# NVlabs/STEP

Hardware: NVIDIA H100
Metric: clips/sec (T=32,224x224) STEP max_iter=3 (higher is better)
Workload: dtype f16

## Files before the change

### include/step_b200.h

```cpp
#ifndef STEP_B200_H_
#define STEP_B200_H_

#include <stddef.h>
#include <stdint.h>

#ifdef __cplusplus
extern "C" {
#endif

typedef struct CUstream_st* step_stream_t;

enum { STEP_F32 = 0, STEP_F16 = 1 };
enum { STEP_OK = 0, STEP_E_ARG = 10001, STEP_E_UNSUPPORTED = 10002, STEP_E_WORKSPACE = 10003,
       STEP_E_DRIVER = 10004 };

int step_version(void);
const char* step_last_error(void);
uint64_t step_launch_count(void);

size_t step_nms_workspace_bytes(int n);
int step_nms_f32(const float* boxes , const float* scores , int n, float thr, int ge,
                 int64_t* keep_out , int* n_keep, void* workspace, size_t ws_bytes,
                 step_stream_t stream);
int step_nms_segmented_f32(const float* boxes, const float* scores, const int* seg_offsets, int n_seg,
// ... 81 lines not shown
  long long noise;
} step_aug_erase;
int step_frames_to_clip_aug_u8(const step_frame_src* table, const step_clip_aug* params, const step_aug_erase* erase,
                               const float* noise, int B, int T, int H, int W, int scale_mode, const float* mean3,
                               const float* std3, float* out, step_stream_t stream);

enum { STEP_A_AUTO = 0, STEP_A_LINEAR = 1, STEP_A_BOX = 2, STEP_A_IM2COL = 3, STEP_A_HALO = 4, STEP_A_BEST = 5,
       STEP_A_SIMT = 9 };
typedef struct {
  int dtype;
  int N, T, H, W;
  int Cin, in_ld;
  int Cout, out_ld, out_coff;
  int KT, KH, KW;
  int ST, SH, SW;
  int PT, PH, PW;
  int OT, OH, OW;
  int relu;
  int w_ld;
  const void* x;
  const void* w;
  const float* scale;
  const float* shift;
  const void* residual;
  int res_ld, res_coff;
  void* y;
  int a_mode;
  int n_splits;
  int split[2];
  void* y_extra[2];
  int ld_extra[2];
  int coff_extra[2];
  int zero_cin_last_kt;
} step_conv_params;
int step_conv3d_fwd(const step_conv_params* p, step_stream_t stream);
int step_debug_tma_tile(const step_conv_params* p, int m_tile, int kt, int kh, int kw, int c0, void* out, int* bk_out,
                        int* box_out, step_stream_t stream);

int step_maxpool3d_fwd(const void* x, int dtype, int N, int T, int H, int W, int C, int in_ld, int KT,
                       int KH, int KW, int ST, int SH, int SW, int PT, int PH, int PW, int pad_hi_t,
                       int pad_hi_h, int pad_hi_w, int OT, int OH, int OW, void* y, int out_ld,
                       step_stream_t stream);
int step_mean_mid(const void* x, int dtype, int A, int B, int P, int C, int ld, void* y, int out_dtype,
                  step_stream_t stream);
int step_mean_mid_strided(const void* x, int dtype, int A, int B, int P, int C, int ld, long long a_stride, void* y,
                          int out_dtype, step_stream_t stream);
size_t step_linear_small_n_workspace_bytes(int M, int K, int N);
int step_linear_small_n(const void* x, int dtype, int M, int K, int x_ld, const void* w, const float* bias,
                        int N, float* y, int y_ld, int act, int accumulate, const int32_t* row_map,
                        void* workspace, size_t ws_bytes, step_stream_t stream);

int step_head_regress(const void* x, int dtype, int R, int T, int K, int x_ld, const void* w12, const float* bias12,
                      int s0, int s1, int e0, int e1, float* local_loc, float* first, float* last, void* workspace,
                      size_t ws_bytes, step_stream_t stream);

int step_bottleneck_exit_f16(const void* h, long long h_ld, const void* w3, const void* x, long long x_ld, const void* w1,
                             const float* shift2, int relu2, void* y, long long y_ld, void* z, long long z_ld, long long M,
                             int planes, int inplanes, int outplanes, step_stream_t stream);

int step_head_losses_f32(const float* logits, const float* local_loc, const float* first_loc, const float* last_loc,
                         const float* tubes, const float* targets, int N, int cls, int T_len, int T, int Tc, float w_loc,
                         float w_nb, float* loss_cls, float* loss_loc, float* loss_nb, int* flags, float* dlogits,
                         float* dloc, float* dfirst, float* dlast, float* scratch, step_stream_t stream);
int step_cls_loss_f32(const float* logits, const float* targets, int N, int cls, float* loss_cls, int* flags, float* dlogits,
                      step_stream_t stream);
int step_roi_align_bwd_nhwc(const void* grad_out, int dtype, int out_ld, const float* rois, int R, float scale, int ph,
// ... 233 lines not shown
```

### step_b200/csrc/conv_umma.cu

```cuda
#include <cuda.h>
#include <stdlib.h>
#include <string.h>

#include "common.cuh"
#include "umma_ptx.cuh"

namespace step {

constexpr int kBM = 128;
constexpr int kMaxBN = 256;
constexpr int kStages = 8;
constexpr int kThreads = 384;
constexpr int kConsumers = 256;
constexpr int kCopyThreads = 96;
constexpr int kPersistMaxKBlocks = 100;
constexpr int kBookBytes = 2 * kStages * 8 + 2 * 8 + 2 * 2 * kMaxBN * 4;
constexpr int kProducerRegs = 40, kConsumerRegs = 232;

#define STEP_CONV_TILES(X)                                                                                         \
  X(64, 32) X(64, 64) X(64, 128) X(64, 144) X(64, 152) X(64, 176) X(64, 192) X(64, 208) X(64, 224) X(64, 256)      \
  X(32, 64) X(32, 128) X(32, 144) X(32, 152) X(32, 160) X(32, 208) X(32, 224)                                      \
  X(16, 64)

__host__ __device__ constexpr int staging_pitch(int BN) { return ((BN / 8 + 1) | 1) * 16; }

struct ConvGeom {
  int mode;
  int taps, KT, KH, KW, PT, PH, PW;
  int kblocks_per_tap;
  int BN, n_tiles;
  int n_stages;
  int n_splits, split[2], ld_extra[2], coff_extra[2];
  __half* y_extra[2];
  int Cout, out_ld, out_coff, res_ld, res_coff, relu;
  int OT, OH, OW, Nimg;
  long long M;
  int tiles;
  int bw, bh, bt, tiles_w, tiles_h, tiles_t;
  int a_bytes;
};

__device__ __forceinline__ long long tile_row_pixel(const ConvGeom& g, int m_tile, int row) {
  if (g.mode == STEP_A_BOX) {
    int r = m_tile;
    const int bw0 = (r % g.tiles_w) * g.bw; r /= g.tiles_w;
    const int bh0 = (r % g.tiles_h) * g.bh; r /= g.tiles_h;
    const int bt0 = (r % g.tiles_t) * g.bt; const int bn = r / g.tiles_t;
    const int dw = row % g.bw, rr = row / g.bw;
    const int dh = rr % g.bh, dt = rr / g.bh;
    const int ow = bw0 + dw, oh = bh0 + dh, ot = bt0 + dt;
    if (dt < g.bt && ow < g.OW && oh < g.OH && ot < g.OT) return (((long long)bn * g.OT + ot) * g.OH + oh) * g.OW + ow;
    return -1;
  }
  const long long m = (long long)m_tile * kBM + row;
  return m < g.M ? m : -1;
}

__device__ __forceinline__ bool mbar_try_wait(uint64_t* bar, uint32_t parity) {
  uint32_t done;
  asm volatile("{\n\t.reg .pred p;\n\tmbarrier.try_wait.parity.shared::cta.b64 p, [%1], %2;\n\tselp.u32 %0, 1, 0, p;\n\t}"
               : "=r"(done) : "r"(smem_u32(bar)), "r"(parity) : "memory");
  return done != 0;
}

template <int BK, int BN>
__global__ void __launch_bounds__(kThreads, 1)
conv_umma_kernel(const __grid_constant__ CUtensorMap map_a, const __grid_constant__ CUtensorMap map_b, ConvGeom g,
                 const float* __restrict__ scale, const float* __restrict__ shift, const __half* __restrict__ residual,
                 __half* __restrict__ y) {
  static_assert(BN % 8 == 0 && BN <= kMaxBN, "wgmma N is a multiple of 8, at most 256");
  constexpr bool kRealloc = BN > 128;
  constexpr bool kBulkOut = BN > 128;
  constexpr int kABytes = kBM * BK * 2;
  constexpr int kBBytes = BN * BK * 2;
  extern __shared__ __align__(1024) uint8_t smem_raw[];
  uint64_t* full_bar = (uint64_t*)smem_raw;
  uint64_t* empty_bar = full_bar + kStages;
  uint64_t* out_full = empty_bar + kStages;
  uint64_t* out_empty = out_full + 1;
  float* s_consts = (float*)(out_empty + 1);
  uint8_t* smem = (uint8_t*)(((uintptr_t)smem_raw + kBookBytes + 1023) & ~(uintptr_t)1023);
  uint8_t* sA = smem;
  uint8_t* sB = smem + g.n_stages * kABytes;
  uint8_t* stg = smem + g.n_stages * (kABytes + kBBytes);
  constexpr int pitch = staging_pitch(BN);

  const int warp = threadIdx.x >> 5, lane = threadIdx.x & 31;
  const int num_kb = g.taps * g.kblocks_per_tap;

  if (threadIdx.x == 0) {
    prefetch_tensormap(&map_a);
    prefetch_tensormap(&map_b);
    for (int s = 0; s < kStages; ++s) { mbar_init(&full_bar[s], 1); mbar_init(&empty_bar[s], 2); }
    mbar_init(out_full, kConsumers / 32);
    mbar_init(out_empty, kCopyThreads / 32);
    fence_barrier_init();
  }
  auto stage_consts = [&](int n_tile, int buf, int t, int nthr) {
    float* s_scale = s_consts + buf * 2 * kMaxBN;
    float* s_shift = s_scale + kMaxBN;
    for (int i = t; i < BN; i += nthr) {
      const int c = n_tile * BN + i;
      s_scale[i] = (scale && c < g.Cout) ? scale[c] : 1.0f;
      s_shift[i] = (shift && c < g.Cout) ? shift[c] : 0.0f;
    }
  };
  if (threadIdx.x < 128) stage_consts(blockIdx.x % g.n_tiles, 0, threadIdx.x, 128);
  __syncthreads();

  if (warp < 4) {
    if constexpr (kRealloc) setmaxnreg_dec<kProducerRegs>();
    if (warp == 0) {
      if (elect_one()) {
        const uint32_t tx_bytes = (uint32_t)(g.a_bytes + kBBytes);
        int stage = 0; uint32_t phase = 0;
        for (int tile = blockIdx.x; tile < g.tiles; tile += gridDim.x) {
          const int m_tile = tile / g.n_tiles, n0 = (tile - m_tile * g.n_tiles) * BN;
          long long m0 = (long long)m_tile * kBM;
          int bn = 0, bt0 = 0, bh0 = 0, bw0 = 0;
          if (g.mode == STEP_A_BOX) {
            int r = m_tile;
            bw0 = (r % g.tiles_w) * g.bw; r /= g.tiles_w;
            bh0 = (r % g.tiles_h) * g.bh; r /= g.tiles_h;
            bt0 = (r % g.tiles_t) * g.bt; bn = r / g.tiles_t;
          }
          int iw = 0, ih = 0, it = 0, in_ = 0;
          if (g.mode == STEP_A_IM2COL) {
            long long r = m0;
            iw = (int)(r % g.OW); r /= g.OW;
            ih = (int)(r % g.OH); r /= g.OH;
            it = (int)(r % g.OT); in_ = (int)(r / g.OT);
            iw -= g.PW; ih -= g.PH; it -= g.PT;
          }
          int kw = 0, kh = 0, kt = 0;
          for (int tap = 0; tap < g.taps; ++tap) {
            for (int kc = 0; kc < g.kblocks_per_tap; ++kc) {
              mbar_wait(&empty_bar[stage], phase ^ 1);
              mbar_expect_tx(&full_bar[stage], tx_bytes);
              const int c0 = kc * BK;
              uint8_t* a_dst = sA + stage * kABytes;
              if (g.mode == STEP_A_LINEAR) {
                tma_load_2d(&map_a, &full_bar[stage], a_dst, c0, (int)m0);
              } else if (g.mode == STEP_A_BOX) {
                tma_load_5d(&map_a, &full_bar[stage], a_dst, c0, bw0 + kw - g.PW, bh0 + kh - g.PH, bt0 + kt - g.PT, bn);
              } else {
                tma_load_im2col_5d(&map_a, &full_bar[stage], a_dst, c0, iw, ih, it, in_, (uint16_t)kw, (uint16_t)kh,
                                   (uint16_t)kt);
              }
              tma_load_3d(&map_b, &full_bar[stage], sB + stage * kBBytes, c0, tap, n0);
              if (++stage == g.n_stages) { stage = 0; phase ^= 1; }
            }
            if (++kw == g.KW) { kw = 0; if (++kh == g.KH) { kh = 0; ++kt; } }
          }
        }
      }
    } else {
      const int ct = threadIdx.x - 32;
      int i_tile = 0;
      for (int tile = blockIdx.x; tile < g.tiles; tile += gridDim.x, ++i_tile) {
        const int m_tile = tile / g.n_tiles, n0 = (tile - m_tile * g.n_tiles) * BN;
        if (tile + (int)gridDim.x < g.tiles) stage_consts((tile + gridDim.x) % g.n_tiles, (i_tile + 1) & 1, ct, kCopyThreads);
        while (!mbar_try_wait(out_full, i_tile & 1)) __nanosleep(128);
        if constexpr (!kBulkOut) {
          constexpr int cpr = BN / 8;
          constexpr int kUnroll = 4;
          for (int i0 = ct; i0 < kBM * cpr; i0 += kUnroll * kCopyThreads) {
            uint4 val[kUnroll];
#pragma unroll
            for (int u = 0; u < kUnroll; ++u) {
              const int i = i0 + u * kCopyThreads, rr = i / cpr, ch = i - rr * cpr;
              if (i < kBM * cpr) val[u] = *reinterpret_cast<const uint4*>(stg + (size_t)rr * pitch + ch * 16);
            }
#pragma unroll
            for (int u = 0; u < kUnroll; ++u) {
              const int i = i0 + u * kCopyThreads, rr = i / cpr, ch = i - rr * cpr;
              const int col = n0 + ch * 8;
              if (i >= kBM * cpr || col >= g.Cout) continue;
              const long long rp = tile_row_pixel(g, m_tile, rr);
              if (rp < 0) continue;
              __half* dst = y + (size_t)rp * g.out_ld + g.out_coff + col;
              if (g.n_splits > 0 && col >= g.split[0]) {
                const int d = (g.n_splits > 1 && col >= g.split[1]) ? 1 : 0;
                dst = g.y_extra[d] + (size_t)rp * g.ld_extra[d] + g.coff_extra[d] + (col - g.split[d]);
              }
              *reinterpret_cast<uint4*>(dst) = val[u];
            }
          }
          __syncwarp();
          if (lane == 0) mbar_arrive(out_empty);
          continue;
        }
        const int end = min(n0 + BN, g.Cout);
        for (int rr = ct; rr < kBM; rr += kCopyThreads) {
          const long long rp = tile_row_pixel(g, m_tile, rr);
          if (rp < 0) continue;
          for (int col = n0; col < end;) {
            __half* dst = y + (size_t)rp * g.out_ld + g.out_coff + col;
            int next = end;
            if (g.n_splits > 0) {
              if (col >= g.split[0]) {
                const int d = (g.n_splits > 1 && col >= g.split[1]) ? 1 : 0;
                dst = g.y_extra[d] + (size_t)rp * g.ld_extra[d] + g.coff_extra[d] + (col - g.split[d]);
                if (d == 0 && g.n_splits > 1) next = min(end, g.split[1]);
              } else {
                next = min(end, g.split[0]);
              }
            }
            bulk_store(dst, stg + (size_t)rr * pitch + (col - n0) * 2, (uint32_t)(next - col) * 2);
            col = next;
          }
        }
        bulk_commit();
        bulk_wait_read<0>();
        __syncwarp();
        if (lane == 0) mbar_arrive(out_empty);
      }
    }
  } else {
    if constexpr (kRealloc) setmaxnreg_inc<kConsumerRegs>();
    const int wg = (warp >> 2) - 1;
    const int ct = threadIdx.x - 128;
    const uint64_t hi = desc_hi_kmajor<BK>();
    const uint64_t a_lo0 = desc_lo(sA + wg * 64 * BK * 2), b_lo0 = desc_lo(sB);
    const int wrow = wg * 64 + (warp & 3) * 16 + (lane >> 2);
    float acc[BN / 2];
    int stage = 0; uint32_t phase = 0;
    int i_tile = 0;
    for (int tile = blockIdx.x; tile < g.tiles; tile += gridDim.x, ++i_tile) {
      const int m_tile = tile / g.n_tiles, n0 = (tile - m_tile * g.n_tiles) * BN;
#pragma unroll
      for (int i = 0; i < BN / 2; ++i) acc[i] = 0.0f;
      int prev = -1;
      for (int kb = 0; kb < num_kb; ++kb) {
        mbar_wait(&full_bar[stage], phase);
        const uint64_t a_lo = a_lo0 + (uint64_t)(stage * (kABytes >> 4)), b_lo = b_lo0 + (uint64_t)(stage * (kBBytes >> 4));
        wg_fence();
#pragma unroll
        for (int k = 0; k < BK / 16; ++k)
          wgmma_f16<BN>(acc, hi | (a_lo + 2 * k), hi | (b_lo + 2 * k), 1u);
        wg_commit();
        wg_wait<1>();
        if (prev >= 0 && ct % 128 == 0) mbar_arrive(&empty_bar[prev]);
        prev = stage;
        if (++stage == g.n_stages) { stage = 0; phase ^= 1; }
      }
      wg_wait<0>();
      if (ct % 128 == 0) mbar_arrive(&empty_bar[prev]);
      mbar_wait(out_empty, (i_tile & 1) ^ 1);
      const float* s_scale = s_consts + (i_tile & 1) * 2 * kMaxBN;
      const float* s_shift = s_scale + kMaxBN;
#pragma unroll
      for (int i = 0; i < 2; ++i) {
        const int row = wrow + 8 * i;
        const long long pix = residual ? tile_row_pixel(g, m_tile, row) : -1;
        const __half* rrow = pix >= 0 ? residual + (size_t)pix * g.res_ld + g.res_coff + n0 : nullptr;
        uint8_t* srow = stg + (size_t)row * pitch;
#pragma unroll
        for (int j = 0; j < BN / 8; ++j) {
          const int col = 8 * j + 2 * (lane & 3);
          float f0 = fmaf(acc[4 * j + 2 * i], s_scale[col], s_shift[col]);
          float f1 = fmaf(acc[4 * j + 2 * i + 1], s_scale[col + 1], s_shift[col + 1]);
// ... 25 lines not shown
  __syncwarp();
  if (threadIdx.x == 0) {
    long long m0 = (long long)m_tile * kBM;
    mbar_expect_tx(&bar, (uint32_t)g.a_bytes);
    if (g.mode == STEP_A_LINEAR) {
      tma_load_2d(&map_a, &bar, smem, c0, (int)m0);
    } else if (g.mode == STEP_A_BOX) {
      int r = m_tile;
      int bw0 = (r % g.tiles_w) * g.bw; r /= g.tiles_w;
      int bh0 = (r % g.tiles_h) * g.bh; r /= g.tiles_h;
      int bt0 = (r % g.tiles_t) * g.bt; int bn = r / g.tiles_t;
      tma_load_5d(&map_a, &bar, smem, c0, bw0 + kw - g.PW, bh0 + kh - g.PH, bt0 + kt - g.PT, bn);
    } else {
      long long r = m0;
      int iw = (int)(r % g.OW); r /= g.OW;
      int ih = (int)(r % g.OH); r /= g.OH;
      int it = (int)(r % g.OT); int in_ = (int)(r / g.OT);
      tma_load_im2col_5d(&map_a, &bar, smem, c0, iw - g.PW, ih - g.PH, it - g.PT, in_, (uint16_t)kw, (uint16_t)kh, (uint16_t)kt);
    }
  }
  mbar_wait(&bar, 0);
  __syncwarp();
  for (int i = threadIdx.x; i < kABytes / 4; i += 32) ((uint32_t*)out)[i] = ((uint32_t*)smem)[i];
}

static int pick_bk(int Cin) {
  if (Cin <= 16) return 16;
  const int k64 = (Cin + 63) / 64 * 64, k32 = (Cin + 31) / 32 * 32;
  return k32 < k64 ? 32 : 64;
}

struct ConvTile {
  int BK, BN;
  void (*kernel)(CUtensorMap, CUtensorMap, ConvGeom, const float*, const float*, const __half*, __half*);
};
static const ConvTile kTiles[] = {
#define STEP_TILE_ENTRY(bk, bn) {bk, bn, conv_umma_kernel<bk, bn>},
    STEP_CONV_TILES(STEP_TILE_ENTRY)
#undef STEP_TILE_ENTRY
};
constexpr int kNumTiles = (int)(sizeof(kTiles) / sizeof(kTiles[0]));

static int pick_tile(int BK, int Cout) {
  int best = -1; long best_pad = 0, best_n = 0;
  for (int i = 0; i < kNumTiles; ++i) {
    if (kTiles[i].BK != BK) continue;
    const long n = (Cout + kTiles[i].BN - 1) / kTiles[i].BN, pad = n * kTiles[i].BN - Cout;
    if (best < 0 || pad < best_pad || (pad == best_pad && n < best_n)) { best = i; best_pad = pad; best_n = n; }
  }
  return best;
}

static void pick_box(int OW, int OH, int OT, int* bw, int* bh, int* bt) {
  double best = -1;
  for (int w = 1; w <= OW && w <= kBM; ++w)
    for (int h = 1; h <= OH && w * h <= kBM; ++h) {
      int t = kBM / (w * h);
      if (t > OT) t = OT;
      if (t < 1) continue;
      double eff = ((double)OW / (((OW + w - 1) / w) * w)) * ((double)OH / (((OH + h - 1) / h) * h)) *
                   ((double)OT / (((OT + t - 1) / t) * t)) * ((double)(w * h * t) / kBM);
      if (eff > best + 1e-9) { best = eff; *bw = w; *bh = h; *bt = t; }
    }
}

static std::atomic<int> g_two_ctas[kNumTiles];
static std::atomic<unsigned long long> g_attr_seen[kNumTiles];
// ... 115 lines not shown
  }
  if (rc) return rc;
  if ((rc = encode_weights3d(&pl->map_b, p->w, p->Cout, taps, p->Cin, p->w_ld, BK, g.BN, swizzle_for(BK),
                             CU_TENSOR_MAP_L2_PROMOTION_L2_256B, "conv3d(f16): B")))
    return rc;
  STEP_CHECK_ARG(m_tiles * g.n_tiles < (1LL << 31), "conv3d(f16): grid too large");
  g.tiles = (int)(m_tiles * g.n_tiles);
  const long per_stage = (long)kBM * BK * 2 + (long)g.BN * BK * 2;
  const long fixed = kBookBytes + 1024 + (long)kBM * staging_pitch(g.BN);
  int st = (int)((113L * 1024 - fixed) / per_stage);
  if (st > kStages) st = kStages;
  bool two = false;
  if (st >= 3) {
    if (int rc = two_ctas_fit(pl->tile, (size_t)(fixed + st * per_stage), &two)) return rc;
  }
  if (!two) st = (int)((227L * 1024 - fixed) / per_stage);
  g.n_stages = st > kStages ? kStages : st;
  STEP_CHECK_ARG(g.n_stages >= 2, "conv3d(f16): tile does not fit shared memory");
  pl->smem_bytes = (size_t)(fixed + g.n_stages * per_stage);
  int sms = 0;
  if (int rc = sm_count(&sms)) return rc;
  const long resident = (long)sms * (two ? 2 : 1);
  const bool persist = g.taps * g.kblocks_per_tap <= kPersistMaxKBlocks && g.tiles > resident;
  pl->grid = dim3((unsigned)(persist ? resident : g.tiles));
  return 0;
}

int conv3d_umma_launch(const step_conv_params* p, step_stream_t stream) {
  ConvPlan pl;
  if (int rc = build_plan(p, &pl)) return rc;
  const ConvTile& t = kTiles[pl.tile];
  if (int rc = allow_dynamic_smem(t.kernel, g_attr_seen[pl.tile], 227 * 1024, "conv_umma_kernel")) return rc;
  return launch_tc("conv_umma_kernel", t.kernel, pl.grid, kThreads, pl.smem_bytes, cu(stream), pl.map_a, pl.map_b, pl.g,
                   p->scale, p->shift, (const __half*)p->residual, (__half*)p->y);
}

}

using namespace step;

extern "C" int step_debug_tma_tile(const step_conv_params* p, int m_tile, int kt, int kh, int kw, int c0, void* out,
                                   int* bk_out, int* box_out , step_stream_t stream) {
  ConvPlan pl;
  if (int rc = build_plan(p, &pl)) return rc;
  if (bk_out) *bk_out = pl.BK;
  if (box_out) { box_out[0] = pl.g.bw; box_out[1] = pl.g.bh; box_out[2] = pl.g.bt; }
  size_t smem = 1024 + (size_t)kBM * pl.BK * 2;
  if (pl.BK == 64) tma_dump_kernel<64><<<1, 32, smem, cu(stream)>>>(pl.map_a, pl.g, m_tile, kt, kh, kw, c0, (uint8_t*)out);
  else if (pl.BK == 32) tma_dump_kernel<32><<<1, 32, smem, cu(stream)>>>(pl.map_a, pl.g, m_tile, kt, kh, kw, c0, (uint8_t*)out);
  else tma_dump_kernel<16><<<1, 32, smem, cu(stream)>>>(pl.map_a, pl.g, m_tile, kt, kh, kw, c0, (uint8_t*)out);
  STEP_LAUNCH_CHECK("tma_dump_kernel");
  return 0;
}
```

### step_b200/engine.py

```python
import contextlib
import math
import os

import torch

from . import _lib as L

A_MODE = {"box": L.A_BOX, "im2col": L.A_IM2COL, "auto": L.A_AUTO, "simt": L.A_SIMT, "best": L.A_BEST}[
    os.environ.get("STEP_B200_AMODE", "best")]


RECORDER = None
TAPE = None
DEBUG_SYNC = os.environ.get("STEP_B200_DEBUG_SYNC", "0") == "1"
STEM_HALO = os.environ.get("STEP_B200_STEM_HALO", "1") != "0"


BRANCH_STREAMS = os.environ.get("STEP_B200_BRANCH_STREAMS", "1") != "0"
FUSE_1X1 = os.environ.get("STEP_B200_FUSE_1X1", "1") != "0"
_side_streams = {}


@contextlib.contextmanager
def recording(tape):
    global TAPE, BRANCH_STREAMS
    saved = TAPE, BRANCH_STREAMS
    TAPE = tape
    if tape is not None:
        BRANCH_STREAMS = False
    try:
        yield tape
    finally:
        TAPE, BRANCH_STREAMS = saved


def side_streams(device, n=3):
    key = (device.type, device.index, torch.cuda.current_stream(device).cuda_stream)
    st = _side_streams.get(key)
    if st is None or len(st) < n:
        st = [torch.cuda.Stream(device=device) for _ in range(n)]
        _side_streams[key] = st
    return st[:n]


def run_parallel(device, main_fn, side_fns, first_side=0):
    if not BRANCH_STREAMS or not side_fns:
        main_fn()
        for f in side_fns:
            f()
        return
    cur = torch.cuda.current_stream(device)
    fork = cur.record_event()
    streams = side_streams(device, first_side + len(side_fns))[first_side:]
    joins = []
    for st, f in zip(streams, side_fns):
        st.wait_event(fork)
        with torch.cuda.stream(st):
            f()
            joins.append(st.record_event())
    main_fn()
    for ev in joins:
        cur.wait_event(ev)


def torch_dtype(code):
    return torch.float16 if code == L.F16 else torch.float32


def dtype_code(fp16):
    env = os.environ.get("STEP_B200_PRECISION")
    if env:
        return {"fp16": L.F16, "fp32": L.F32}[env]
    return L.F16 if fp16 else L.F32


class Act:
    __slots__ = ("buf", "C", "coff")

    def __init__(self, buf, C=None, coff=0):
        assert buf.dim() == 5 and buf.is_contiguous()
        self.buf = buf
        self.C = buf.shape[4] - coff if C is None else C
        self.coff = coff

    @staticmethod
    def empty(N, T, H, W, C, code, device, ld=None):
        return Act(torch.empty((N, T, H, W, ld or C), dtype=torch_dtype(code), device=device), C, 0)

    N = property(lambda s: s.buf.shape[0])
    T = property(lambda s: s.buf.shape[1])
    H = property(lambda s: s.buf.shape[2])
    W = property(lambda s: s.buf.shape[3])
    ld = property(lambda s: s.buf.shape[4])
    code = property(lambda s: L.dt(s.buf))
    device = property(lambda s: s.buf.device)
# ... 197 lines not shown
        out_dims = same_out_dims((x.T, x.H, x.W), k, stride)
    p = L.step_conv_params()
    p.dtype = code
    p.N, p.T, p.H, p.W = x.N, x.T, x.H, x.W
    p.Cin, p.in_ld = x.C, x.ld
    p.Cout, p.out_ld, p.out_coff = out.C + sum(e.C for e in (extra_outs or [])), out.ld, out.coff
    if extra_outs:
        p.n_splits = len(extra_outs)
        edge = out.C
        for i, e in enumerate(extra_outs):
            p.split[i] = edge
            p.y_extra[i] = e.buf.data_ptr()
            p.ld_extra[i], p.coff_extra[i] = e.ld, e.coff
            edge += e.C
    p.KT, p.KH, p.KW = k
    p.ST, p.SH, p.SW = stride
    p.PT, p.PH, p.PW = pad_lo
    p.OT, p.OH, p.OW = out_dims
    p.relu = 1 if relu else 0
    p.w_ld = w_packed.shape[2]
    p.x = x.data_ptr()
    p.w = w_packed.data_ptr()
    p.scale = scale.data_ptr() if scale is not None else None
    p.shift = shift.data_ptr() if shift is not None else None
    if residual is not None:
        p.residual = residual.buf.data_ptr()
        p.res_ld, p.res_coff = residual.ld, residual.coff
    p.y = out.buf.data_ptr()
    p.zero_cin_last_kt = int(zero_cin_last_kt)
    p.a_mode = A_MODE if a_mode is None else a_mode
    if p.a_mode in (L.A_BOX, L.A_IM2COL, L.A_BEST) and k == (1, 1, 1):
        p.a_mode = L.A_AUTO
    assert (out.N, out.T, out.H, out.W) == (x.N,) + tuple(out_dims), "conv: output buffer shape mismatch"
    L.check(L.lib().step_conv3d_fwd(p, L.stream()))
    if DEBUG_SYNC:
        try:
            torch.cuda.synchronize()
        except Exception:
            print("conv fault:", {f: getattr(p, f) for f, _ in p._fields_ if isinstance(getattr(p, f), int)}, flush=True)
            raise
    if TAPE is not None:
        TAPE.append(dict(kind="conv", x=x, w=w_packed, scale=scale, out=out, extra_outs=list(extra_outs or []), k=tuple(k),
                         stride=tuple(stride), pad_lo=tuple(pad_lo), relu=bool(relu), residual=residual, tag=tag))
    if RECORDER is not None:
        RECORDER.append((p, (x.buf, w_packed, scale, shift, out.buf, residual.buf if residual is not None else None,
                             [e.buf for e in (extra_outs or [])])))
    return out


def pool_out(size, k, s):
    lo, hi = same_pad(k, s)
    P = size + lo + hi
    o = -(-(P - k) // s) + 1
    if (o - 1) * s >= P:
        o -= 1
    return o, lo, hi


def maxpool(x, k, s, out=None):
    (ot, pt, ht), (oh, ph, hh), (ow, pw, hw) = (pool_out(d, kk, ss) for d, kk, ss in zip((x.T, x.H, x.W), k, s))
    if out is None:
        out = Act.empty(x.N, ot, oh, ow, x.C, x.code, x.device)
    L.check(L.lib().step_maxpool3d_fwd(L.c_void_p(x.data_ptr()), x.code, x.N, x.T, x.H, x.W, x.C, x.ld, k[0], k[1],
                                       k[2], s[0], s[1], s[2], pt, ph, pw, ht, hh, hw, ot, oh, ow,
                                       L.c_void_p(out.data_ptr()), out.ld, L.stream()))
    if TAPE is not None:
        TAPE.append(dict(kind="pool", x=x, out=out, k=tuple(k), stride=tuple(s), pad_lo=(pt, ph, pw), pad_hi=(ht, hh, hw)))
    return out


def mean_mid(x_ptr, code, A, B, P, C, ld, device, out_code=L.F32):
    y = torch.empty((A, P * C), dtype=torch_dtype(out_code), device=device)
    L.check(L.lib().step_mean_mid(L.c_void_p(x_ptr), code, A, B, P, C, ld, L.ptr(y), out_code, L.stream()))
    return y


def linear_small_n(x, M, K, x_ld, w, bias, N, y=None, act=0, accumulate=False, row_map=None):
    if y is None:
        y = torch.empty((M, N), dtype=torch.float32, device=x.device)
# ... 7 lines not shown
```

### step_b200/inference.py

```python
import numpy as np
import torch

from . import _lib as L
from . import engine as E
from .engine import Act
from .networks import act_of, to_act
from .tube_utils import flatten_tubes, tube_update


def _ext_mode(args, i):
    if i < args.max_iter and args.NUM_CHUNKS[i + 1] == args.NUM_CHUNKS[i] + 2:
        return {"predict": L.EXT_PREDICT, "extrapolate": L.EXT_EXTRAPOLATE}.get(args.temporal_mode, L.EXT_MEAN)
    return L.EXT_NONE


def stage_tubes(tubes, device):
    flat_np, tubes_nums = flatten_tubes(tubes, batch_idx=True)
    flat = torch.from_numpy(np.ascontiguousarray(flat_np, dtype=np.float32)).to(device)
    clip_of_tube = torch.from_numpy(np.repeat(np.arange(len(tubes_nums)), tubes_nums).astype(np.int32)).to(device)
    return flat, clip_of_tube, tubes_nums


def inference_device(args, feat, ctx_all, nets, exec_iter, flat, clip_of_tube, tubes_nums):
    dev = feat.device
    code = feat.code
    B, T_total = feat.N, feat.T
    R = flat.shape[0]
    roi_net = nets['roi_net']
    history, steps = [], []
    width, height = float(args.image_size[0]), float(args.image_size[1])
    decode_nb = args.temporal_mode == "predict"
    with torch.cuda.device(dev):
        for i in range(1, exec_iter + 1):
            chunks = args.NUM_CHUNKS[i]
            T_start = int((args.NUM_CHUNKS[args.max_iter] - chunks) / 2) * args.T
            T_len = chunks * args.T
            if flat.shape[1] != T_len:
                raise RuntimeError("inference: tubes have %d frames but step %d pools %d" % (flat.shape[1], i, T_len))
            head = nets['det_net%d' % (i - 1)]
            ps = head.pool_size
            cat = Act.empty(R, T_len, ps, ps, 832 + head.fc_dim, code, dev)
            roi_net.pool_into(feat, flat, cat.frames().slice(0, 832), T_len, T_total, T_start)
            ctx_mean = None
            if ctx_all is not None:
                sl = ctx_all[:, T_start:T_start + T_len].contiguous()
                ctx_mean = E.mean_mid(sl.data_ptr(), L.F32, B, T_len, 1, sl.shape[2], sl.shape[2], dev)
            hdev = torch.device(head.device) if getattr(head, "device", None) not in (None, "cpu") else dev
            if hdev.type == "cuda" and hdev.index is None:
                hdev = torch.device("cuda", torch.cuda.current_device())
            if hdev != dev:
                cat_h = Act(cat.buf.to(hdev))
                cm = ctx_mean.to(hdev) if ctx_mean is not None else None
                with torch.cuda.device(hdev):
                    outs = head.forward_act(cat_h, cm, clip_of_tube.to(hdev))
                prob, loc, first, last = (o.to(dev) for o in outs)
            else:
                prob, loc, first, last = head.forward_act(cat, ctx_mean, clip_of_tube)
            ext = _ext_mode(args, i)
            pred_loc, pf, pl, flat_next = tube_update(flat, loc, first if decode_nb else None,
                                                      last if decode_nb else None, clip_of_tube, args.T, decode_nb,
                                                      ext, width, height)
            pred_prob = prob.view(-1, 1, args.num_classes).expand(-1, T_len, -1)
            history.append({'pred_prob': pred_prob, 'pred_loc': pred_loc, 'pred_first_loc': pf, 'pred_last_loc': pl,
                            'tubes_nums': tubes_nums})
            steps.append((flat_next, prob))
            flat = flat_next
    return history, steps


def inference(args, conv_feat, context_feat, nets, exec_iter, tubes, want_trajectory=True):
    L.need_cuda(conv_feat)
    dev = conv_feat.device
    code = E.dtype_code(nets['det_net0'].fp16)
    feat = act_of(conv_feat)
    if feat is None or feat.code != code:
        feat = to_act(conv_feat, code)
    flat, clip_of_tube, tubes_nums = stage_tubes(tubes, dev)
    ctx_all = None
    if not args.no_context:
        L.need_cuda(context_feat)
        ctx_all = context_feat.detach().float().reshape(feat.N, context_feat.shape[1], feat.T).permute(0, 2, 1).contiguous()
    history, steps = inference_device(args, feat, ctx_all, nets, exec_iter, flat, clip_of_tube, tubes_nums)

    trajectory = []
    if want_trajectory:
        for (flat_next, prob), h in zip(steps, history):
            props = flat_next[:, :, 1:].cpu().numpy()
            cls = torch.argmax(prob, dim=-1).cpu()
            T_len = h['pred_loc'].shape[1]
            cur, s = [], 0
            for n in tubes_nums:
                cur.append((props[s:s + n], cls[s:s + n].view(-1, 1).expand(-1, T_len)))
                s += n
            trajectory.append(cur)
    return history, trajectory
```

### step_b200/networks.py

```python
import os

import torch
import torch.nn as nn
import torch.nn.init as init

from . import _lib as L
from . import engine as E
from .engine import Act
from .i3d import build_trunk_stages, set_bn_eval, set_freeze_stats
from .roi_layers import ROIAlign, ROIPool


def weights_init(m):
    if isinstance(m, (nn.Conv2d, nn.Linear, nn.Conv3d)):
        init.xavier_normal_(m.weight.data)
        if m.bias is not None:
            init.constant_(m.bias.data, 0.0)


def act_of(t):
    if t.dim() != 5:
        return None
    phys = t.permute(0, 1, 3, 4, 2)
    if phys.is_contiguous():
# ... 61 lines not shown
                L.ptr(flat_tubes), R, 1.0 / 16.0, ps, ps]
        if self.pool_mode == 'align':
            args.append(0)
        args += [L.c_void_p(out.data_ptr()), out.ld, roi_T, feat_T, t_start]
        if self.pool_mode == 'align':
            args.append(0 if feat.code == L.F16 else 1)
        if argmax is not None:
            args.append(L.ptr(argmax))
        args.append(L.stream())
        L.check(fn(*args))
        return out


class BaseNet(nn.Module):

    def __init__(self, cfg):
        super(BaseNet, self).__init__()
        self.base_name = cfg.base_net
        self.kinetics_pretrain = cfg.kinetics_pretrain
        self.freeze_stats = cfg.freeze_stats
        self.freeze_affine = cfg.freeze_affine
        self.fp16 = cfg.fp16
        if self.base_name == "i3d":
            self.base_model = build_base_i3d(self.kinetics_pretrain, self.freeze_affine)
        else:
            raise NotImplementedError
        set_freeze_stats(self.base_model, self.freeze_stats)

    def forward(self, x):
        L.need_cuda(x)
        with torch.cuda.device(x.device):
            return self.forward_act(x).logical()

    def forward_act(self, x):
        L.need_cuda(x)
        if x.dim() != 5:
            raise RuntimeError("BaseNet: expected [N,T,C,H,W]")
        code = E.dtype_code(self.fp16)
        N, T, C, H, W = x.shape
        src = x.detach().to(torch.float32).contiguous()
        m = self.base_model
        if code == L.F16 and T % 2 == 0 and H % 2 == 0 and W % 2 == 0 and C == 3:
            s2d = Act.empty(N, T // 2, H // 2, W // 2, 32, L.F16, x.device)
            L.check(L.lib().step_clip_to_s2d_f16(L.ptr(src), N, T, C, H, W, L.ptr(s2d.buf), 32, L.stream()))
            a = m[0].forward_s2d(s2d)
        else:
            if code == L.F16:
                raise RuntimeError("BaseNet(fp16): T, H, W must be even and C == 3")
            cp = (C + 3) // 4 * 4
            a = Act.empty(N, T, H, W, cp, code, x.device)
            L.check(L.lib().step_clip_to_ndhwc(L.ptr(src), N, T, C, H, W, L.ptr(a.buf), code, cp, L.stream()))
            a = m[0](a)
        for i in range(1, len(m)):
            a = m[i](a)
        return a

    def train(self, mode=True):
        nn.Module.train(self, mode)
        if mode and self.freeze_stats:
            set_bn_eval(self.base_model)
        return self


def build_base_i3d(kinetics_pretrain=None, freeze_affine=True):
    stages = build_trunk_stages()
    base_model = nn.Sequential(*stages)
# ... 22 lines not shown
```

### step_b200/runner.py

```python
import torch

from . import _lib as L
from . import engine as E
from .inference import inference_device, stage_tubes
from .postprocess import Detector
from .transforms import frame_entry, frame_table


class StepRunner:
    def __init__(self, cfg, nets, B, T_in, H, W, tubes, device=None, context=False, use_graph=True, warmup=2,
                 detect=None, transform=None, source_hw=None):
        self.cfg, self.nets = cfg, nets
        self.device = device or torch.device("cuda", torch.cuda.current_device())
        self.context = context and not cfg.no_context
        self.x = torch.zeros((B, T_in, 3, H, W), dtype=torch.float32, device=self.device)
        self.transform = transform
        if transform is not None:
            if source_hw is None:
                raise ValueError("StepRunner: a transform needs source_hw = (H0, W0)")
            if tuple(transform.size) != (W, H):
                raise ValueError("StepRunner: transform size %s is not the clip's (W, H) = %s" % (transform.size, (W, H)))
            self.src = torch.zeros((B, T_in, 3) + tuple(source_hw), dtype=torch.uint8, device=self.device)
            self.table = frame_table([frame_entry(self.src[b], W) for b in range(B)], self.device)
        self.flat, self.clip_of_tube, self.tubes_nums = stage_tubes(tubes, self.device)
        self.graph = None
        self.history = None
        self.detections = None
        self.detectors = {}
        if detect is not None:
            for i in detect.get("steps", [cfg.max_iter - 1]):
                self.detectors[i] = Detector(self.tubes_nums, cfg.num_classes, self.device, detect["conf_thresh"],
                                             detect["nms_thresh"], W, H, topk=detect.get("topk", 0))
        if not use_graph:
            return
        side = torch.cuda.Stream(device=self.device)
        side.wait_stream(torch.cuda.current_stream(self.device))
        with torch.cuda.stream(side):
            for _ in range(warmup):
                self._body()
        torch.cuda.current_stream(self.device).wait_stream(side)
        torch.cuda.synchronize(self.device)
        g = torch.cuda.CUDAGraph()
        with torch.cuda.graph(g):
            self.history = self._body()
        self.graph = g

    def _body(self):
        with torch.no_grad():
            if self.transform is not None:
                self.transform.launch(self.table, self.x.shape[0], self.x.shape[1], self.x)
            feat = self.nets["base_net"].forward_act(self.x)
            ctx_all = self.nets["context_net"].forward_act(feat) if self.context else None
            hist, _ = inference_device(self.cfg, feat, ctx_all, self.nets, self.cfg.max_iter, self.flat,
                                       self.clip_of_tube, self.tubes_nums)
            if self.detectors:
                self.detections = {i: d.run(hist[i]["pred_prob"], hist[i]["pred_loc"]) for i, d in self.detectors.items()}
        return hist

    def __call__(self, clips=None):
        if self.transform is not None:
            if clips is not None:
                self._stage_frames(clips)
        elif clips is not None and clips.data_ptr() != self.x.data_ptr():
            self.x.copy_(clips, non_blocking=True)
        if self.graph is None:
            return self._body()
        self.graph.replay()
        return self.history

    def _stage_frames(self, frames):
        clips = list(frames) if isinstance(frames, (list, tuple)) else [frames[b] for b in range(frames.shape[0])]
        want = tuple(self.src.shape[1:])
        if len(clips) != self.src.shape[0] or any(tuple(c.shape) != want or c.dtype != torch.uint8 for c in clips):
            raise ValueError("StepRunner: expected %d uint8 clips %s (the captured source size), got %s" % (
                self.src.shape[0], want, [(c.dtype, tuple(c.shape)) for c in clips]))
        if isinstance(frames, torch.Tensor):
            self.src.copy_(frames, non_blocking=True)
        else:
            for dst, c in zip(self.src, clips):
# ... 2 lines not shown
```

### step_b200/training.py

```python
import contextlib
import ctypes

import torch

from . import _lib as L


def head_losses(logits, local_loc, first_loc, last_loc, tubes, targets, T, lambda_reg=5.0, lambda_neighbor=1.0,
                want_grads=False):
    dev = L.same_device(logits, local_loc, first_loc, last_loc, tubes, targets)
    f32 = lambda t: t.detach().to(torch.float32).contiguous()
    logits, local_loc, first_loc, last_loc, tubes, targets = map(f32, (logits, local_loc, first_loc, last_loc, tubes, targets))
    N, cls = logits.shape
    T_len, Tc = local_loc.shape[1], first_loc.shape[1]
    if targets.shape != (N, 3, 6 + cls) or tubes.shape != (N, T_len, 5):
        raise RuntimeError("head_losses: targets %s / tubes %s do not match N=%d, T'=%d, classes=%d"
                           % (tuple(targets.shape), tuple(tubes.shape), N, T_len, cls))
    with torch.cuda.device(dev):
        loss_cls = torch.empty((N * cls,), dtype=torch.float32, device=dev)
        loss_loc = torch.empty((1,), dtype=torch.float32, device=dev)
        loss_nb = torch.empty((1,), dtype=torch.float32, device=dev)
        flags = torch.empty((3,), dtype=torch.int32, device=dev)
        scratch = torch.empty((N * 12,), dtype=torch.float32, device=dev)
        g = None
        if want_grads:
            g = {"logits": torch.empty_like(logits), "local_loc": torch.empty_like(local_loc),
                 "first_loc": torch.empty_like(first_loc), "last_loc": torch.empty_like(last_loc)}
        L.check(L.lib().step_head_losses_f32(L.ptr(logits), L.ptr(local_loc), L.ptr(first_loc), L.ptr(last_loc), L.ptr(tubes),
                                             L.ptr(targets), N, cls, T_len, int(T), Tc, float(lambda_reg), float(lambda_neighbor),
                                             L.ptr(loss_cls), L.ptr(loss_loc), L.ptr(loss_nb), L.ptr(flags),
                                             L.ptr(g["logits"]) if g else None, L.ptr(g["local_loc"]) if g else None,
                                             L.ptr(g["first_loc"]) if g else None, L.ptr(g["last_loc"]) if g else None,
                                             L.ptr(scratch), L.stream()))
        if int(flags[0].item()) == 0:
            loss_cls = torch.zeros((1,), dtype=torch.float32, device=dev)
    return (loss_cls, loss_loc, loss_nb) if not want_grads else (loss_cls, loss_loc, loss_nb, g)


# ... 162 lines not shown
    try:
        yield
    finally:
        e1.record()
        TIMING.setdefault(name, []).append((e0, e1))


def timing_summary():
    torch.cuda.synchronize()
    return {k: round(sum(a.elapsed_time(b) for a, b in v), 2) for k, v in (TIMING or {}).items()}


def trainable_bn(tag):
    bn = getattr(tag, "batch3d", None) if getattr(tag, "use_bn", False) else None
    if bn is None or not (bn.weight.requires_grad or bn.bias.requires_grad):
        return None
    return bn


def check_bn_affine(nets):
    bns = [("%s.%s" % (key, name), m) for key, mod in nets.items() if mod is not None for name, m in mod.named_modules()
           if isinstance(m, torch.nn.BatchNorm3d) and (m.weight.requires_grad or m.bias.requires_grad)]
    if not bns:
        return
    with torch.no_grad():
        bad = torch.stack([((m.weight == 0) & (m.bias > 0)).any() for _, m in bns]).cpu()
    if bool(bad.any()):
        name = bns[int(bad.nonzero()[0, 0])][0]
        raise ValueError("BatchNorm %s has a channel with gamma == 0 and beta > 0: its output is constant and gamma's gradient "
                         "cannot be recovered from it; freeze that layer's affine parameters or give gamma a non-zero value"
                         % name)


def tape_backward(tape, grads, loss_scale=1.0, need_input_grad=None):
    from . import engine as E
    from .engine import Act
    out = {}
    lib = L.lib()
    inv = 1.0 / float(loss_scale)

    def add(param, g):
        out[param] = out[param] + g if param in out else g

    for e in reversed(tape):
        f16 = e["x"].code == L.F16
        if e["kind"] == "pool":
            x, y = e["x"], e["out"]
            gy, gx = grads.of(y), grads.of(x)
            k, s, pl, ph = e["k"], e["stride"], e["pad_lo"], e["pad_hi"]
            ws = torch.empty((y.N * y.T * y.H * y.W * y.C,), dtype=torch.uint8, device=x.device)
            pool_bwd = lib.step_maxpool3d_bwd_f16 if f16 else lib.step_maxpool3d_bwd_f32
            with _phase("pool_bwd"):
                L.check(pool_bwd(L.c_void_p(x.data_ptr()), x.ld, L.c_void_p(gy.data_ptr()), gy.ld, x.N, x.T, x.H,
                                                   x.W, x.C, k[0], k[1], k[2], s[0], s[1], s[2], pl[0], pl[1], pl[2], ph[0], ph[1],
                                                   ph[2], y.T, y.H, y.W, L.c_void_p(gx.data_ptr()), gx.ld, L.ptr(ws), L.stream()))
            continue
        x, w, k = e["x"], e["w"], e["k"]
        strided = e["stride"] != (1, 1, 1)
        if strided and (f16 or need_input_grad is None or need_input_grad(e)):
            raise NotImplementedError("tape_backward: a strided convolution has a weight gradient on the fp32 path only, and no "
                                      "input gradient (the trunk's stem needs none)")
        outs = [e["out"]] + e["extra_outs"]
        y0 = e["out"]
        M = y0.N * y0.T * y0.H * y0.W
        n_total = sum(o.C for o in outs)
        dz = torch.empty((y0.N, y0.T, y0.H, y0.W, n_total), dtype=x.buf.dtype, device=x.device)
# ... 550 lines not shown
```

### step_b200/two_branch.py

```python
import torch
import torch.nn as nn

from . import _lib as L
from . import engine as E
from .engine import Act
from .i3d import I3D_head, set_bn_eval, set_freeze_stats
from .networks import to_act, weights_init

__all__ = ['ContextNet', 'TwoBranchNet']


def build_conv(base_name='i3d', kinetics_pretrain=None, mode='global', freeze_affine=True):
    if base_name != "i3d":
        raise NotImplementedError
    i3d = I3D_head()
    if kinetics_pretrain is not None:
        import os
        if not os.path.isfile(kinetics_pretrain):
            raise ValueError("Kinetics_pretrain doesn't exist: {}".format(kinetics_pretrain))
        model_dict = i3d.state_dict()
        pre = torch.load(kinetics_pretrain, map_location="cpu")
        model_dict.update({k: v for k, v in pre.items() if k in model_dict})
        i3d.load_state_dict(model_dict)
    if mode == 'context':
# ... 60 lines not shown
        self.conv2 = nn.Conv2d(inplanes, planes, kernel_size=1, bias=False)
        self.conv3 = nn.Conv2d(planes, planes, kernel_size=3, stride=stride, padding=1, bias=False)
        self.conv4 = nn.Conv2d(planes, outplanes, kernel_size=1, bias=False)
        self.relu = nn.ReLU(inplace=True)
        self.stride = stride

    def forward(self, x):
        box = {}
        E.run_parallel(x.device,
                       lambda: box.__setitem__("o", conv2d(self.conv3, conv2d(self.conv2, x, True), True)),
                       [lambda: box.__setitem__("res", conv2d(self.conv1, x, False))])
        return conv2d(self.conv4, box["o"], True, residual=box["res"])


class ContextNet(nn.Module):

    def __init__(self, cfg):
        super(ContextNet, self).__init__()
        self.T = cfg.T
        self.freeze_stats = cfg.freeze_stats
        self.freeze_affine = cfg.freeze_affine
        self.fp16 = cfg.fp16
        self.i3d_conv_context = build_conv(cfg.base_net, cfg.kinetics_pretrain, 'context', self.freeze_affine)
        set_freeze_stats(self.i3d_conv_context, self.freeze_stats)
        self.avg_pool = nn.AvgPool3d((1, 13, 13), (1, 1, 1))
        self._init_net()

    def forward(self, conv_feat):
        L.need_cuda(conv_feat)
        with torch.cuda.device(conv_feat.device):
            ctx = self.forward_act(to_act(conv_feat, E.dtype_code(self.fp16)))
        return ctx.permute(0, 2, 1).unsqueeze(-1).unsqueeze(-1)

    def forward_act(self, a, keep=None):
        x = self.i3d_conv_context[0](a)
        x = self.i3d_conv_context[1](x)
        x = self.i3d_conv_context[2](x)
        if keep is not None:
            keep["mixed_5c"] = x
        y = E.mean_mid(x.data_ptr(), x.code, x.N * x.T, x.H * x.W, 1, x.C, x.ld, x.device)
        return y.view(x.N, x.T, x.C)

    def _init_net(self):
        pass

    def set_device(self, device):
        self.device = device

    def train(self, mode=True):
        nn.Module.train(self, mode)
        if mode and self.freeze_stats:
            set_bn_eval(self.i3d_conv_context)
        return self


class TwoBranchNet(nn.Module):

    def __init__(self, cfg, cls_only=False):
        super(TwoBranchNet, self).__init__()
        self.num_classes = cfg.num_classes
        self.T = cfg.T
        self.base_net = cfg.base_net
        self.freeze_stats = cfg.freeze_stats
        self.freeze_affine = cfg.freeze_affine
        self.fc_dim = cfg.fc_dim
        self.dropout_prob = cfg.dropout
# ... 47 lines not shown
    def forward(self, global_feat, context_feat=None, tubes=None, targets=None):
        dev = self.device
        if dev is not None and str(dev) != "cpu":
            global_feat = global_feat.to(dev)
            if context_feat is not None:
                context_feat = context_feat.to(dev)
        L.same_device(global_feat, context_feat)
        code = E.dtype_code(self.fp16)
        N, T, C, W, H = global_feat.shape
        with torch.cuda.device(global_feat.device):
            cat = Act.empty(N, T, W, H, C + self.fc_dim, code, global_feat.device)
            src = to_act(global_feat, code)
            cat.buf[..., :C].copy_(src.buf[..., src.coff:src.coff + C])
            ctx_mean = None
            if context_feat is not None:
                cf = context_feat.detach().float().contiguous().view(N * context_feat.shape[1], T)
                ctx_mean = E.mean_mid(cf.data_ptr(), L.F32, N * context_feat.shape[1], T, 1, 1, 1, cf.device).view(N, -1)
            if targets is None:
                prob, loc, first, last = self.forward_act(cat, ctx_mean, None)
            else:
                prob, loc, first, last, logits = self.forward_act(cat, ctx_mean, None, want_logits=True)
        z = torch.tensor(0., device=prob.device)
        if targets is None:
            return prob, loc, first, last, z.view(-1), z.view(-1), z.view(-1)
        from . import training
        if tubes is None:
            raise RuntimeError("TwoBranchNet.forward: targets need tubes")
        tb, tg = tubes.to(prob.device), targets.to(prob.device)
        if self.cls_only:
            return prob, loc, first, last, training.cls_loss(logits, tg), z.view(-1), z.view(-1)
        lc, ll, ln = training.head_losses(logits, loc, first, last, tb, tg, self.T)
        return prob, loc, first, last, lc, ll, ln

    def forward_act(self, cat, ctx_mean=None, ctx_row_map=None, want_logits=False, keep=None, dropout=None):
        R, T, ps = cat.N, cat.T, self.pool_size
        code = cat.code
        roi = cat.slice(0, 832)
        g = self.i3d_conv[0](roi)
        g = self.i3d_conv[1](g)
        w, bias = _packed(self.downsample, code)
        gconv = cat.slice(832, self.fc_dim)
        E.conv(g, w, None, bias, gconv, (1, 1, 1), relu=False, tag=self.downsample)
        hw = self._head_weights()
        D = self.fc_dim * ps * ps
        gsrc = gconv
        if dropout is not None:
            gsrc = Act.empty(R, T, ps, ps, self.fc_dim, code, cat.device)
            ctx_cols = 0 if hw["ctx_w"] is None else hw["ctx_w"].shape[1]
            L.check(L.lib().step_dropout_global_fwd(dropout[0], L.c_void_p(gconv.data_ptr()), code, cat.ld, R, T, ps * ps, self.fc_dim,
                                                    ctx_cols, L.c_void_p(gsrc.data_ptr()), gsrc.ld, L.stream()))
        xbar = E.mean_mid(gsrc.data_ptr(), code, R, T, ps * ps, self.fc_dim, gsrc.ld, cat.device)
        has_ctx = ctx_mean is not None and hw["ctx_w"] is not None
        logits = E.linear_small_n(xbar, R, D, D, hw["cls_w"], hw["cls_b"], self.num_classes,
                                  act=0 if has_ctx else 1)
        if has_ctx:
            E.linear_small_n(ctx_mean, R, 1024, 1024, hw["ctx_w"], None, self.num_classes, y=logits, act=1,
                             accumulate=True, row_map=ctx_row_map)
        prob = logits
        raw = None
        if want_logits:
            raw = E.linear_small_n(xbar, R, D, D, hw["cls_w"], hw["cls_b"], self.num_classes, act=0)
            if has_ctx:
                E.linear_small_n(ctx_mean, R, 1024, 1024, hw["ctx_w"], None, self.num_classes, y=raw, act=0,
                                 accumulate=True, row_map=ctx_row_map)
        if self.cls_only:
            if keep is not None:
# ... 87 lines not shown
```

Measured before the change: 1162.

## Schedule persistent conv tiles dynamically with a global atomic tile counter

Result: no change. 1169, median of 6 (+0.7%).

```diff
diff --git a/include/step_b200.h b/include/step_b200.h
--- a/include/step_b200.h
+++ b/include/step_b200.h
@@ -137,6 +137,7 @@
   int ld_extra[2];
   int coff_extra[2];
   int zero_cin_last_kt;
+  unsigned int* tile_counter;
 } step_conv_params;
 int step_conv3d_fwd(const step_conv_params* p, step_stream_t stream);
 int step_debug_tma_tile(const step_conv_params* p, int m_tile, int kt, int kh, int kw, int c0, void* out, int* bk_out,
diff --git a/step_b200/csrc/conv_umma.cu b/step_b200/csrc/conv_umma.cu
--- a/step_b200/csrc/conv_umma.cu
+++ b/step_b200/csrc/conv_umma.cu
@@ -14,7 +14,9 @@
 constexpr int kConsumers = 256;
 constexpr int kCopyThreads = 96;
 constexpr int kPersistMaxKBlocks = 100;
-constexpr int kBookBytes = 2 * kStages * 8 + 2 * 8 + 2 * 2 * kMaxBN * 4;
+constexpr int kTileRing = kStages;
+constexpr int kTileReaders = kConsumers / 32 + kCopyThreads / 32;
+constexpr int kBookBytes = 2 * kStages * 8 + 2 * 8 + 2 * 2 * kMaxBN * 4 + 2 * kTileRing * 8 + kTileRing * 4;
 constexpr int kProducerRegs = 40, kConsumerRegs = 232;
 
 #define STEP_CONV_TILES(X)                                                                                         \
@@ -63,11 +65,25 @@
   return done != 0;
 }
 
+__device__ __forceinline__ int next_tile(unsigned int* counter, int tile, int tiles) {
+  if (!counter) return tile + (int)gridDim.x;
+  const int t = (int)gridDim.x + (int)atomicAdd(counter, 1u);
+  if (t >= tiles) {
+    __threadfence();
+    if (atomicAdd(counter + 1, 1u) == gridDim.x - 1) {
+      __threadfence();
+      counter[0] = 0u;
+      counter[1] = 0u;
+    }
+  }
+  return t;
+}
+
 template <int BK, int BN>
 __global__ void __launch_bounds__(kThreads, 1)
 conv_umma_kernel(const __grid_constant__ CUtensorMap map_a, const __grid_constant__ CUtensorMap map_b, ConvGeom g,
                  const float* __restrict__ scale, const float* __restrict__ shift, const __half* __restrict__ residual,
-                 __half* __restrict__ y) {
+                 __half* __restrict__ y, unsigned int* __restrict__ tile_counter) {
   static_assert(BN % 8 == 0 && BN <= kMaxBN, "wgmma N is a multiple of 8, at most 256");
   constexpr bool kRealloc = BN > 128;
   constexpr bool kBulkOut = BN > 128;
@@ -79,6 +95,9 @@
   uint64_t* out_full = empty_bar + kStages;
   uint64_t* out_empty = out_full + 1;
   float* s_consts = (float*)(out_empty + 1);
+  uint64_t* tid_full = (uint64_t*)(s_consts + 2 * 2 * kMaxBN);
+  uint64_t* tid_empty = tid_full + kTileRing;
+  int* tile_ids = (int*)(tid_empty + kTileRing);
   uint8_t* smem = (uint8_t*)(((uintptr_t)smem_raw + kBookBytes + 1023) & ~(uintptr_t)1023);
   uint8_t* sA = smem;
   uint8_t* sB = smem + g.n_stages * kABytes;
@@ -94,8 +113,18 @@
     for (int s = 0; s < kStages; ++s) { mbar_init(&full_bar[s], 1); mbar_init(&empty_bar[s], 2); }
     mbar_init(out_full, kConsumers / 32);
     mbar_init(out_empty, kCopyThreads / 32);
+    for (int s = 0; s < kTileRing; ++s) { mbar_init(&tid_full[s], 1); mbar_init(&tid_empty[s], kTileReaders); }
     fence_barrier_init();
-  }
+    tile_ids[0] = blockIdx.x;
+    mbar_arrive(&tid_full[0]);
+  }
+  auto take_tile = [&](int i) {
+    mbar_wait(&tid_full[i % kTileRing], (uint32_t)(i / kTileRing) & 1);
+    const int t = tile_ids[i % kTileRing];
+    __syncwarp();
+    if (lane == 0) mbar_arrive(&tid_empty[i % kTileRing]);
+    return t;
+  };
   auto stage_consts = [&](int n_tile, int buf, int t, int nthr) {
     float* s_scale = s_consts + buf * 2 * kMaxBN;
     float* s_shift = s_scale + kMaxBN;
@@ -114,7 +143,7 @@
       if (elect_one()) {
         const uint32_t tx_bytes = (uint32_t)(g.a_bytes + kBBytes);
         int stage = 0; uint32_t phase = 0;
-        for (int tile = blockIdx.x; tile < g.tiles; tile += gridDim.x) {
+        for (int i = 0, tile = blockIdx.x, next; tile < g.tiles; ++i, tile = next) {
           const int m_tile = tile / g.n_tiles, n0 = (tile - m_tile * g.n_tiles) * BN;
           long long m0 = (long long)m_tile * kBM;
           int bn = 0, bt0 = 0, bh0 = 0, bw0 = 0;
@@ -152,14 +181,19 @@
             }
             if (++kw == g.KW) { kw = 0; if (++kh == g.KH) { kh = 0; ++kt; } }
           }
+          const int slot = (i + 1) % kTileRing;
+          mbar_wait(&tid_empty[slot], ((uint32_t)((i + 1) / kTileRing) & 1) ^ 1);
+          next = next_tile(tile_counter, tile, g.tiles);
+          tile_ids[slot] = next;
+          mbar_arrive(&tid_full[slot]);
         }
       }
     } else {
       const int ct = threadIdx.x - 32;
-      int i_tile = 0;
-      for (int tile = blockIdx.x; tile < g.tiles; tile += gridDim.x, ++i_tile) {
+      for (int i_tile = 0, tile = take_tile(0), next; tile < g.tiles; ++i_tile, tile = next) {
         const int m_tile = tile / g.n_tiles, n0 = (tile - m_tile * g.n_tiles) * BN;
-        if (tile + (int)gridDim.x < g.tiles) stage_consts((tile + gridDim.x) % g.n_tiles, (i_tile + 1) & 1, ct, kCopyThreads);
+        next = take_tile(i_tile + 1);
+        if (next < g.tiles) stage_consts(next % g.n_tiles, (i_tile + 1) & 1, ct, kCopyThreads);
         while (!mbar_try_wait(out_full, i_tile & 1)) __nanosleep(128);
         if constexpr (!kBulkOut) {
           constexpr int cpr = BN / 8;
@@ -225,8 +259,9 @@
     const int wrow = wg * 64 + (warp & 3) * 16 + (lane >> 2);
     float acc[BN / 2];
     int stage = 0; uint32_t phase = 0;
-    int i_tile = 0;
-    for (int tile = blockIdx.x; tile < g.tiles; tile += gridDim.x, ++i_tile) {
+    for (int i_tile = 0;; ++i_tile) {
+      const int tile = take_tile(i_tile);
+      if (tile >= g.tiles) break;
       const int m_tile = tile / g.n_tiles, n0 = (tile - m_tile * g.n_tiles) * BN;
 #pragma unroll
       for (int i = 0; i < BN / 2; ++i) acc[i] = 0.0f;
@@ -318,7 +353,7 @@
 
 struct ConvTile {
   int BK, BN;
-  void (*kernel)(CUtensorMap, CUtensorMap, ConvGeom, const float*, const float*, const __half*, __half*);
+  void (*kernel)(CUtensorMap, CUtensorMap, ConvGeom, const float*, const float*, const __half*, __half*, unsigned int*);
 };
 static const ConvTile kTiles[] = {
 #define STEP_TILE_ENTRY(bk, bn) {bk, bn, conv_umma_kernel<bk, bn>},
@@ -500,7 +535,7 @@
   const ConvTile& t = kTiles[pl.tile];
   if (int rc = allow_dynamic_smem(t.kernel, g_attr_seen[pl.tile], 227 * 1024, "conv_umma_kernel")) return rc;
   return launch_tc("conv_umma_kernel", t.kernel, pl.grid, kThreads, pl.smem_bytes, cu(stream), pl.map_a, pl.map_b, pl.g,
-                   p->scale, p->shift, (const __half*)p->residual, (__half*)p->y);
+                   p->scale, p->shift, (const __half*)p->residual, (__half*)p->y, p->tile_counter);
 }
 
 }
diff --git a/step_b200/engine.py b/step_b200/engine.py
--- a/step_b200/engine.py
+++ b/step_b200/engine.py
@@ -1,4 +1,5 @@
 import contextlib
+import functools
 import math
 import os
 
@@ -61,6 +62,42 @@
     main_fn()
     for ev in joins:
         cur.wait_event(ev)
+
+
+COUNTER_SLOTS = 512
+_counters = None
+
+
+@contextlib.contextmanager
+def tile_counters():
+    global _counters
+    if _counters is not None:
+        yield
+        return
+    _counters = {}
+    try:
+        yield
+    finally:
+        _counters = None
+
+
+def counted(fn):
+    @functools.wraps(fn)
+    def wrapper(*args, **kwargs):
+        with tile_counters():
+            return fn(*args, **kwargs)
+    return wrapper
+
+
+def _tile_counter(device):
+    key = torch.cuda.current_stream(device).cuda_stream
+    slabs = _counters if _counters is not None else {}
+    ent = slabs.get(key)
+    if ent is None or ent[1] == ent[0].numel() // 2:
+        ent = slabs[key] = [torch.zeros(2 * (COUNTER_SLOTS if _counters is not None else 1), dtype=torch.int32, device=device), 0]
+    slab, i = ent
+    ent[1] = i + 1
+    return slab, slab.data_ptr() + 8 * i
 
 
 def torch_dtype(code):
@@ -324,6 +361,9 @@
     if p.a_mode in (L.A_BOX, L.A_IM2COL, L.A_BEST) and k == (1, 1, 1):
         p.a_mode = L.A_AUTO
     assert (out.N, out.T, out.H, out.W) == (x.N,) + tuple(out_dims), "conv: output buffer shape mismatch"
+    slab = None
+    if code == L.F16:
+        slab, p.tile_counter = _tile_counter(x.device)
     L.check(L.lib().step_conv3d_fwd(p, L.stream()))
     if DEBUG_SYNC:
         try:
@@ -336,7 +376,7 @@
                          stride=tuple(stride), pad_lo=tuple(pad_lo), relu=bool(relu), residual=residual, tag=tag))
     if RECORDER is not None:
         RECORDER.append((p, (x.buf, w_packed, scale, shift, out.buf, residual.buf if residual is not None else None,
-                             [e.buf for e in (extra_outs or [])])))
+                             [e.buf for e in (extra_outs or [])], slab)))
     return out
 
 
diff --git a/step_b200/inference.py b/step_b200/inference.py
--- a/step_b200/inference.py
+++ b/step_b200/inference.py
@@ -21,6 +21,7 @@
     return flat, clip_of_tube, tubes_nums
 
 
+@E.counted
 def inference_device(args, feat, ctx_all, nets, exec_iter, flat, clip_of_tube, tubes_nums):
     dev = feat.device
     code = feat.code
@@ -68,6 +69,7 @@
     return history, steps
 
 
+@E.counted
 def inference(args, conv_feat, context_feat, nets, exec_iter, tubes, want_trajectory=True):
     L.need_cuda(conv_feat)
     dev = conv_feat.device
diff --git a/step_b200/networks.py b/step_b200/networks.py
--- a/step_b200/networks.py
+++ b/step_b200/networks.py
@@ -117,6 +117,7 @@
         with torch.cuda.device(x.device):
             return self.forward_act(x).logical()
 
+    @E.counted
     def forward_act(self, x):
         L.need_cuda(x)
         if x.dim() != 5:
diff --git a/step_b200/runner.py b/step_b200/runner.py
--- a/step_b200/runner.py
+++ b/step_b200/runner.py
@@ -45,6 +45,7 @@
             self.history = self._body()
         self.graph = g
 
+    @E.counted
     def _body(self):
         with torch.no_grad():
             if self.transform is not None:
diff --git a/step_b200/training.py b/step_b200/training.py
--- a/step_b200/training.py
+++ b/step_b200/training.py
@@ -4,6 +4,7 @@
 import torch
 
 from . import _lib as L
+from . import engine as E
 
 
 def head_losses(logits, local_loc, first_loc, last_loc, tubes, targets, T, lambda_reg=5.0, lambda_neighbor=1.0,
@@ -232,6 +233,7 @@
                          % name)
 
 
+@E.counted
 def tape_backward(tape, grads, loss_scale=1.0, need_input_grad=None):
     from . import engine as E
     from .engine import Act
diff --git a/step_b200/two_branch.py b/step_b200/two_branch.py
--- a/step_b200/two_branch.py
+++ b/step_b200/two_branch.py
@@ -116,6 +116,7 @@
             ctx = self.forward_act(to_act(conv_feat, E.dtype_code(self.fp16)))
         return ctx.permute(0, 2, 1).unsqueeze(-1).unsqueeze(-1)
 
+    @E.counted
     def forward_act(self, a, keep=None):
         x = self.i3d_conv_context[0](a)
         x = self.i3d_conv_context[1](x)
@@ -229,6 +230,7 @@
         lc, ll, ln = training.head_losses(logits, loc, first, last, tb, tg, self.T)
         return prob, loc, first, last, lc, ll, ln
 
+    @E.counted
     def forward_act(self, cat, ctx_mean=None, ctx_row_map=None, want_logits=False, keep=None, dropout=None):
         R, T, ps = cat.N, cat.T, self.pool_size
         code = cat.code
```
